# ddiazdom/grlBWT

Hardware: AMD Instinct MI355X
Metric: input MB/s building BCR BWT on 10 GB DNA reads, 1/2/4/8 MI355X (higher is better)
Workload: dtype u8; 1 GPU; 66225166 x 150 bp Illumina-style reads (10000000066 bytes) from a 330000000 bp genome, 0.5% substitutions; BASELINE configs[3]; input_resident=HBM, output=.rl_bwt image in HBM, parallelism=1 GPU

## Files before the change

### grlbwt_amd/csrc/capi_impl.hpp

```cpp
#include "../../include/grlbwt_hip.h"

#include <fcntl.h>
#include <zlib.h>
#include <sys/stat.h>
#include <unistd.h>

#include <atomic>
#include <chrono>
#include <cstdio>
#include <cstring>
#include <condition_variable>
#include <memory>
#include <mutex>
#include <string>
#include <system_error>
#include <thread>
#include <vector>


struct grlbwt_fm {
    uint32_t flags = 0;
    std::unique_ptr<grl32::Engine::FmIndex> f32;
    std::unique_ptr<grl64::Engine::FmIndex> f64;
};
// ... 1411 lines not shown
        for (uint64_t p = 0; p < n; p++) { key[p] = z[p] ? rb[j++] : ra[i++]; at[key[p] + 1]++; }
        for (int c = 0; c < 256; c++) at[c + 1] += at[c];
        for (uint64_t p = 0; p < n; p++) want[at[key[p]]++] = z[p];
    }
    grl32::DBuf<uint8_t> dra(na + 16), drb(nb + 16), dz(n + 16), dp(n + 16), dout(n + 64);
    prim::h2d(dra.p, ra.data(), na); prim::h2d(drb.p, rb.data(), nb); prim::h2d(dz.p, z.data(), n); prim::h2d(dp.p, prev.data(), n);
    prim::dev_memset(dout.p, 0xA5, n + 64);
    typename E::MergeRound W;
    W.alloc(n);
    if (W.changed(dz.p, dp.p, na) != exp_changed) return 1;
    if (W.changed(dz.p, nullptr, na) != 0) return 2;
    W.step(dra.p, drb.p, dz.p, dout.p);
    prim::sync();
    const std::vector<uint8_t> got = dout.to_host(n + 64);
    for (uint64_t p = 0; p < n; p++)
        if (got[p] != want[p]) {
            fprintf(stderr, "[grlbwt] selftest merge round: %d-byte index, %llu rows (%llu of A), %u symbols: row %llu expected flag %u, got %u\n", ib,
                    (unsigned long long)n, (unsigned long long)na, sigma, (unsigned long long)p, want[p], got[p]);
            return 3;
        }
    for (uint64_t p = n; p < n + 64; p++) if (got[p] != 0xA5) return 4;
    return 0;
}
int test_merge_round(uint64_t n, uint64_t seed) {
    const uint64_t m = self_size(n);
    const uint32_t sigmas[3] = {2, 5, 256};
    for (int k = 0; k < 3; k++) {
        if (int rc = test_merge_round_one<grl32::Engine>(m, seed + k, sigmas[k], 4)) return -(600 + rc);
        if (int rc = test_merge_round_one<grl64::Engine>(m + 1 + k, seed + 10 + k, sigmas[k], 8)) return -(610 + rc);
    }
    return 0;
}

int selftest(uint64_t n, uint64_t seed) {
    if (n < 2) n = 2;
    std::vector<uint32_t> h(n);
    uint64_t s = seed;
    for (uint64_t i = 0; i < n; i++) h[i] = (uint32_t)sm64(s);
    grl32::DBuf<uint32_t> d(n);
    prim::h2d(d.p, h.data(), n * 4);
    {
        grl32::DBuf<uint64_t> o(n + 1);
        uint64_t tot = prim::exclusive_scan<uint64_t>(n, U32In{d.p}, o.p, true, "selftest.scan");
        auto ho = o.to_host(n + 1);
        uint64_t acc = 0;
        for (uint64_t i = 0; i < n; i++) { if (ho[i] != acc) return -1; acc += h[i] & 1023u; }
        if (ho[n] != acc || tot != acc) return -2;
    }
    {
        std::vector<uint32_t> small(n);
        for (uint64_t i = 0; i < n; i++) small[i] = h[i] & 7u;
        grl32::DBuf<uint32_t> o(n);
        prim::h2d(o.p, small.data(), n * 4);
        uint32_t tot = prim::exclusive_scan<uint32_t>(n, prim::PtrIn<uint32_t>{o.p}, o.p, false, "selftest.scan32");
        auto ho = o.to_host(n);
        uint32_t acc = 0;
        for (uint64_t i = 0; i < n; i++) { if (ho[i] != acc) return -3; acc += small[i]; }
        if (tot != acc) return -4;
    }
    {
        uint64_t sum = 0; uint32_t mn = ~0u, mx = 0;
        for (uint64_t i = 0; i < n; i++) { sum += h[i] & 1023u; if (h[i] < mn) mn = h[i]; if (h[i] > mx) mx = h[i]; }
        if (prim::reduce_sum<uint64_t>(n, U32In{d.p}) != sum) return -5;
        if (prim::reduce_min<uint32_t>(n, U32Raw{d.p}) != mn) return -6;
        if (prim::reduce_max<uint32_t>(n, U32Raw{d.p}) != mx) return -7;
    }
// ... 5 lines not shown
        for (uint64_t i = 0; i < n; i++) {
            bool b = (hw[i >> 6] >> (i & 63)) & 1ull;
            if (b != ((h[i] % 3u) == 1u)) return -8;
        }
        if (n % 64) if (hw[nw - 1] >> (n % 64)) return -9;
    }
    {
        uint64_t hist[256], ref[256] = {0};
        const uint8_t *hb = (const uint8_t *)h.data();
        uint64_t nb = n * 4 - 3;
        for (uint64_t i = 0; i < nb; i++) ref[hb[i]]++;
        prim::byte_histogram((const uint8_t *)d.p, nb, hist);
        for (int i = 0; i < 256; i++) if (hist[i] != ref[i]) return -10;
    }
    { int r = test_sort<uint32_t, uint32_t>(n, seed + 1, 19); if (r) return -20 - r; }
    { int r = test_sort<uint64_t, uint32_t>(n, seed + 2, 45); if (r) return -30 - r; }
    { int r = test_sort<uint32_t, uint64_t>(n, seed + 3, 8); if (r) return -40 - r; }
    { int r = test_sort<uint64_t, uint32_t>(n, seed + 4, 3); if (r) return -50 - r; }
    { int r = test_sort<uint64_t, uint64_t>(n, seed + 5, 33); if (r) return -60 - r; }
    { int r = test_sort_keys(n, seed + 6, 21); if (r) return -90 - r; }
    { int r = test_sort<uint64_t, uint32_t>(n, seed + 7, 54); if (r) return -100 - r; }
    { int r = test_sort<uint64_t, uint32_t>(n, seed + 8, 51); if (r) return -110 - r; }
    { int r = test_sort_keys(n, seed + 9, 18); if (r) return -120 - r; }
    { int r = test_sort<uint32_t, uint64_t>(n, seed + 10, 27); if (r) return -130 - r; }
    { int r = test_sort<uint32_t, uint32_t>(n, seed + 11, 20); if (r) return -140 - r; }
    { int r = test_part(n, seed + 12, 6); if (r) return -150 - r; }
    { int r = test_part(n, seed + 13, 11); if (r) return -160 - r; }
    { int r = test_part(n, seed + 14, 18); if (r) return -170 - r; }
    { int r = test_pair_scan<uint32_t, uint32_t>(n, h, d.p); if (r) return -70 - r; }
    { int r = test_pair_scan<uint64_t, uint64_t>(n, h, d.p); if (r) return -80 - r; }
    { int r = test_stream_merge(n, seed); if (r) return r; }
#ifdef GRLBWT_PRIM_HIP
    { int r = test_seg_sort_all(seed + 40); if (r) return r; }
#endif
    { int r = test_pack(); if (r) return r; }
    { int r = test_set_bits(n, seed + 60); if (r) return r; }
    { int r = test_merge_round(n, seed + 80); if (r) return r; }
    return 0;
}

}

extern "C" {

int grlbwt_abi_version(void) { return GRLBWT_ABI_VERSION; }
const char *grlbwt_backend_name(void) { return prim::kIsDevice ? "hip-gfx950" : "serial-test-standin"; }

const char *grlbwt_strerror(int code) {
    switch (code) {
        case GRLBWT_OK: return "ok";
        case GRLBWT_EINVAL: return "invalid argument or call out of order";
        case GRLBWT_EDEVICE: return "HIP device/runtime error";
        case GRLBWT_ENOMEM: return "out of memory";
        case GRLBWT_EILLFORMED: return "Error: the file is ill formed";
        case GRLBWT_ERANGE: return "input beyond the supported range";
        case GRLBWT_ENOSPC: return "phrase table overflow";
        case GRLBWT_EINTERNAL: return "internal consistency check failed";
        case GRLBWT_ENOTDNA: return "The input seems not to be DNA";
        default: return "unknown error";
    }
}
const char *grlbwt_last_error(const grlbwt_ctx *ctx) { return ctx ? ctx->err.c_str() : ""; }

static void warn_env_switches_once() {
    static bool done = false;
    if (done) return;
// ... 87 lines not shown
    if (!ctx || !dev_in || !dev_out) return GRLBWT_EINVAL;
    return guarded(ctx, [&] {
        grl64::Engine::FastxInfo info = grl64::Engine::fastx_to_text((const uint8_t *)dev_in, n_in, (fx_flags & GRLBWT_FASTX_REVCOMP) != 0,
                                                                     (uint8_t *)dev_out, capacity);
        if (n_out) *n_out = info.n_out;
        if (n_strings) *n_strings = info.n_strings;
    });
}
int grlbwt_alphabet_size(const grlbwt_ctx *ctx, uint64_t *n_distinct) {
    if (!HAS_ENG(ctx) || !n_distinct) return GRLBWT_EINVAL;
    *n_distinct = ENG(ctx, alpha_n);
    return GRLBWT_OK;
}
int grlbwt_alphabet_download(const grlbwt_ctx *ctx, uint64_t *values_out) {
    if (!HAS_ENG(ctx) || !values_out || ENG(ctx, alpha_n) == 0) return GRLBWT_EINVAL;
    return guarded(const_cast<grlbwt_ctx *>(ctx), [&] { prim::d2h(values_out, ENG(ctx, alpha.p), ENG(ctx, alpha_n) * 8); });
}
int grlbwt_alphabet_compact_device(grlbwt_ctx *ctx, const void *dev_cells, uint64_t n_cells, int cell_bytes, void *dev_ranks_u32,
                                   void *dev_values_u64, uint64_t capacity_values, uint64_t *n_distinct) {
    if (!ctx || !dev_cells || !dev_ranks_u32 || !dev_values_u64 || n_cells == 0 || !(cell_bytes == 4 || cell_bytes == 8)) return GRLBWT_EINVAL;
    return guarded(ctx, [&] {
        const bool big = n_cells >= kIdx32Limit || (ctx->flags & GRLBWT_FLAG_FORCE_IDX64);
        uint64_t k = big ? grl64::Engine::alphabet_compact_device(dev_cells, n_cells, cell_bytes, (uint32_t *)dev_ranks_u32, (uint64_t *)dev_values_u64, capacity_values)
                         : grl32::Engine::alphabet_compact_device(dev_cells, n_cells, cell_bytes, (uint32_t *)dev_ranks_u32, (uint64_t *)dev_values_u64, capacity_values);
        if (n_distinct) *n_distinct = k;
        if (k > capacity_values) throw prim::Error(GRLBWT_EINVAL, "alphabet compaction: more distinct values than the output buffer holds");
    });
}
int grlbwt_text_load_fastx(grlbwt_ctx *ctx, const char *path, uint32_t fx_flags, uint64_t *n_strings) {
    if (!ctx || !path) return GRLBWT_EINVAL;
    return guarded(ctx, [&] { load_fastx(ctx, path, fx_flags, n_strings); });
}
int grlbwt_text_attach_device(grlbwt_ctx *ctx, const void *dev_cells, uint64_t n_cells, int cell_bytes) {
    if (!ctx || !dev_cells || ((uintptr_t)dev_cells & 15)) return GRLBWT_EINVAL;
    return guarded(ctx, [&] { load(ctx, dev_cells, n_cells, cell_bytes, false); });
}
int grlbwt_get_stats(const grlbwt_ctx *ctx, grlbwt_stats *out) {
    if (!HAS_ENG(ctx) || !out) return GRLBWT_EINVAL;
    if (ctx->e32) fill_stats(*ctx->e32, out); else fill_stats(*ctx->e64, out);
    return GRLBWT_OK;
}

int grlbwt_parse_round(grlbwt_ctx *ctx, grlbwt_round_info *info, int *done) {
    if (!HAS_ENG(ctx)) return GRLBWT_EINVAL;
    return guarded(ctx, [&] {
        bool d = ENG(ctx, parse_round());
        if (done) *done = d ? 1 : 0;
        if (info) { int r = (int)ENG(ctx, levels.size()) - 1; if (ctx->e32) fill_round(*ctx->e32, r, info); else fill_round(*ctx->e64, r, info); }
    });
}
int grlbwt_parse_phase(grlbwt_ctx *ctx, int *n_rounds) {
    if (!HAS_ENG(ctx)) return GRLBWT_EINVAL;
    return guarded(ctx, [&] { int r = ENG(ctx, parse_phase()); if (n_rounds) *n_rounds = r; });
}
int grlbwt_round_info_get(const grlbwt_ctx *ctx, int round, grlbwt_round_info *info) {
    if (!HAS_ENG(ctx) || !info || round < 0 || round >= (int)ENG(ctx, levels.size())) return GRLBWT_EINVAL;
    if (ctx->e32) fill_round(*ctx->e32, round, info); else fill_round(*ctx->e64, round, info);
    return GRLBWT_OK;
}

int grlbwt_induce_first(grlbwt_ctx *ctx) {
    if (!HAS_ENG(ctx)) return GRLBWT_EINVAL;
    return guarded(ctx, [&] { ENG(ctx, first_bwt()); });
}
int grlbwt_induce_level(grlbwt_ctx *ctx, int *level, grlbwt_level_info *info) {
    if (!HAS_ENG(ctx)) return GRLBWT_EINVAL;
    return guarded(ctx, [&] {
// ... 509 lines not shown
```

### grlbwt_amd/csrc/engine_impl.hpp

```cpp

#include "switches.hpp"

namespace GRL_NS {

using prim::u8;
using prim::u16;
using prim::u32;
using prim::u64;
typedef GRL_IDX_T idx_t;

template <class T>
struct DBuf {
    T *p = nullptr;
    u64 n = 0;
    DBuf() {}
    explicit DBuf(u64 n_) { alloc(n_); }
    DBuf(const DBuf &) = delete;
    DBuf &operator=(const DBuf &) = delete;
    DBuf(DBuf &&o) noexcept : p(o.p), n(o.n) { o.p = nullptr; o.n = 0; }
    DBuf &operator=(DBuf &&o) noexcept {
        if (this != &o) { release(); p = o.p; n = o.n; o.p = nullptr; o.n = 0; }
        return *this;
    }
    ~DBuf() { release(); }
    void alloc(u64 n_) { release(); p = (T *)prim::dev_alloc((n_ ? n_ : 1) * sizeof(T)); n = n_; }
    void release() { if (p) prim::dev_free(p); p = nullptr; n = 0; }
    void shrink(u64 n_) { if (p && n_ < n) { prim::dev_shrink(p, (n_ ? n_ : 1) * sizeof(T)); n = n_; } }
    void zero() { prim::dev_memset(p, 0, n * sizeof(T)); }
    void fill_ff() { prim::dev_memset(p, 0xFF, n * sizeof(T)); }
    std::vector<T> to_host(u64 cnt) const { std::vector<T> h(cnt); prim::d2h(h.data(), p, cnt * sizeof(T)); return h; }
    T get(u64 i) const { T v; prim::d2h(&v, p + i, sizeof(T)); return v; }
};

static inline unsigned bitlen64(u64 v) { return v == 0 ? 0 : 64 - (unsigned)__builtin_clzll(v); }

static inline bool test_fail_rank(int fail_rank, int me) {
    if constexpr (prim::kIsDevice) { (void)fail_rank; (void)me; return false; }
    else return fail_rank == me;
}

template <class T>
GRL_HD u64 upper_bound(const T *a, u64 n, T v) {
    u64 lo = 0, hi = n;
    while (lo < hi) { u64 mid = (lo + hi) >> 1; if (a[mid] <= v) lo = mid + 1; else hi = mid; }
    return lo;
}
template <class T>
GRL_HD u64 lower_bound(const T *a, u64 n, T v) {
    u64 lo = 0, hi = n;
    while (lo < hi) { u64 mid = (lo + hi) >> 1; if (a[mid] < v) lo = mid + 1; else hi = mid; }
    return lo;
}

template <class cell_t, bool FIRST>
struct CellOps {
    cell_t sep;
    GRL_HD u32 sym(cell_t c) const { return FIRST ? (u32)c : (u32)(c >> 2); }
    GRL_HD bool rep(cell_t c) const { return FIRST ? true : (bool)((c >> 1) & 1); }
    GRL_HD bool isT(cell_t c) const { return FIRST ? (c == sep) : (bool)(c & 1); }
};

GRL_HD bool bit_at(const u64 *w, u64 i) { return (w[i >> 6] >> (i & 63)) & 1ull; }
GRL_HD u64 next_set_bit(const u64 *w, u64 p, u64 n) {
    u64 r = n;
    if (p < n) {
        u64 wi = p >> 6;
        u64 x = w[wi] >> (p & 63);
        if (x) r = p + (u64)__builtin_ctzll(x);
        else {
            bool found = false;
            for (wi++; !found && (wi << 6) < n; wi++) { x = w[wi]; if (x) { r = (wi << 6) + (u64)__builtin_ctzll(x); found = true; } }
        }
        if (r > n) r = n;
    }
    return r;
}
GRL_HD u64 next_set_bit_far(const u64 *w, u64 p, u64 n) {
    u64 r = n;
    if (p < n) {
        u64 wi = p >> 6;
        u64 x = w[wi] >> (p & 63);
        if (x) r = p + (u64)__builtin_ctzll(x);
        else {
            bool found = false;
            wi++;
            bool fast = true;
            while (fast && ((wi + 8) << 6) <= n) {
                u64 any = 0;
// ... 3074 lines not shown
};

class Engine {
  public:
    ~Engine() { prim::stages_drop(); }
    int cell_bytes = 1;
    const void *text0 = nullptr;
    DBuf<u8> own0;
    DBuf<u32> rank0;
    DBuf<u64> alpha;
    u64 alpha_n = 0;
    u64 sep0() const { return alpha_n ? 0 : stats.min_sym; }
    u64 n0 = 0;
    Stats stats;
    Timers tm;
    std::vector<LevelData> levels;
    std::vector<LevelInfo> linfo;
    DBuf<u32> cur_text;
    u64 cur_n = 0;
    u32 cur_sigma = 0;
    bool parse_done = false;
    Runs bwt;
    int bwt_level = -1;
    DBuf<u8> image;
    u64 sym_present[4] = {0, 0, 0, 0};
    bool sym_present_known = false;
    u64 image_bytes = 0;
    u64 image_runs = 0;
    u64 image_part_off = 0, image_part_bytes = 0;
    bool keep_texts = false;
    std::vector<DBuf<u32>> kept_texts;
    std::vector<Runs> kept_bwts;

    template <class cell_t>
    void stats_t(const cell_t *t, u64 n, const u64 *hist256 = nullptr) {
        StageTimer st(&tm.stats, "stats");
        cell_t sep;
        prim::d2h(&sep, t + (n - 1), sizeof(cell_t));
        u64 mn, mx, F = n;
        if (sizeof(cell_t) == 1) {
            u64 h[256];
            if (hist256) std::memcpy(h, hist256, sizeof h);
            else prim::byte_histogram((const u8 *)t, n, h);
            mn = 0; while (h[mn] == 0) mn++;
            mx = 255; while (h[mx] == 0) mx--;
            F = 0; for (int i = 0; i < 256; i++) if (h[i] > F) F = h[i];
            stats.n_strings = h[(u64)sep];
            for (int i = 0; i < 4; i++) sym_present[i] = 0;
            for (int i = 0; i < 256; i++) if (h[i]) sym_present[i >> 6] |= 1ull << (i & 63);
            sym_present_known = true;
        } else {
            mn = prim::reduce_min<u64>(n, CellIn<cell_t>{t}, "stats.min");
            mx = prim::reduce_max<u64>(n, CellIn<cell_t>{t}, "stats.max");
            stats.n_strings = prim::reduce_sum<u64>(n, EqIn<cell_t>{t, sep}, "stats.nstr");
        }
        if ((u64)sep != mn) throw prim::Error(-84, "Error: the file is ill formed");
        stats.n_syms = n; stats.min_sym = mn; stats.max_sym = mx; stats.max_sym_freq = F;
        if (mx >= (1ull << 30) - 8) {
            if constexpr (sizeof(cell_t) >= 4) {
                rank0.alloc(n + 4);
                alpha_n = alphabet_compact<cell_t>(t, n, mx, rank0.p, alpha);
                if ((const void *)t == (const void *)own0.p) own0.release();
                text0 = rank0.p; cell_bytes = 4;
            }
        }
        stats.sb = (bitlen64(mx + 4) + 7) / 8;
        stats.fb = (bitlen64(F) + 7) / 8;
    }

    void load_text(const void *dev_cells, u64 n, int w, const u64 *hist256 = nullptr) {
        if (n == 0 || !(w == 1 || w == 2 || w == 4 || w == 8)) throw prim::Error(-22, "bad input size or cell width");
        if (sizeof(idx_t) == 4 && n >= 0xFFFFFF00ull) throw prim::Error(-75, "input too large for the 32-bit index build");
        if (n >= kPosMask) throw prim::Error(-75, "input too large");
        cell_bytes = w; text0 = dev_cells; n0 = n;
        prim::rt().tag = -1; prim::rt().phase = 0;
        prim::pool_reserve((size_t)(n * (u64)w) * (sizeof(idx_t) == 4 ? 22 : 30));
        levels.clear(); linfo.clear(); kept_texts.clear(); kept_bwts.clear();
        parse_done = false; bwt_level = -1; image_bytes = 0;
        rank0.release(); alpha.release(); alpha_n = 0;
        tm = Timers();
        switch (w) {
            case 1: stats_t<u8>((const u8 *)dev_cells, n, hist256); break;
            case 2: stats_t<u16>((const u16 *)dev_cells, n); break;
            case 4: stats_t<u32>((const u32 *)dev_cells, n); break;
            default: stats_t<u64>((const u64 *)dev_cells, n); break;
        }
        cur_n = n;
        cur_sigma = alpha_n ? (u32)alpha_n : (u32)(stats.max_sym + 1);
    }
    void upload_text(const void *host_cells, u64 n, int w) {
        own0.alloc(n * (u64)w + 16);
        prim::h2d(own0.p, host_cells, n * (u64)w);
        load_text(own0.p, n, w);
    }

    struct LocalParse {
        u64 n_occ = 0, D = 0, S = 0, cap = 0;
        u32 maxlen = 0;
        DBuf<u32> next_text;
        DBuf<u64> ph_pos; DBuf<idx_t> ph_freq; DBuf<u32> ph_len, ph_slot, ph_off; DBuf<u8> ph_lastT;
        u64 Ds = 0; int part_bits = 0, rec_b = 0; u32 slot0 = 0;
        DBuf<prim::U128> ph_key;
        DBuf<u32> lid, pbase;
        DBuf<u8> ph_vflag;
        DBuf<u64> pstart;
        prim::RecSort psort;
        void clear() {
            n_occ = D = S = cap = Ds = 0; maxlen = 0; part_bits = rec_b = 0; slot0 = 0;
            next_text.release(); ph_pos.release(); ph_freq.release(); ph_len.release(); ph_slot.release(); ph_off.release(); ph_lastT.release();
            ph_key.release(); ph_vflag.release(); pstart.release(); lid.release(); pbase.release(); psort.release();
        }
    };

// ... 1422 lines not shown
        while (bwt_level > 0) induce_level();
    }

    bool image_fused = false;
    void image_header(u32 sb, u32 fb) {
        u8 hdr[16] = {0};
        for (int i = 0; i < 8; i++) { hdr[i] = (u8)((u64)sb >> (8 * i)); hdr[8 + i] = (u8)((u64)fb >> (8 * i)); }
        prim::h2d(image.p, hdr, 16);
    }
    void finish() {
        if (bwt_level != 0) throw prim::Error(-22, "induction not finished");
        prim::rt().tag = -1; prim::rt().phase = 0;
        StageTimer st(&tm.finish, "finish");
        u32 sb = (u32)stats.sb, fb = (u32)stats.fb;
        if (!image_fused) {
        image_bytes = 16 + bwt.R * (u64)(sb + fb);
        image.alloc(image_bytes);
        image_header(sb, fb);
        if (sb + fb <= 8 && fb < 8) prim::pack_records(bwt.R, RunRecordFn{bwt.sym.p, run_len(), sb, alpha.p}, sb + fb, image.p + 16, "pack_rl_bwt");
        else prim::for_each(bwt.R, PackRunsFn{bwt.sym.p, run_len(), sb, fb, image.p, 16u, alpha.p}, "pack_rl_bwt");
        }
        image_fused = false;
        image_runs = bwt.R;
        image_part_off = 0; image_part_bytes = image_bytes;
        prim::sync();
    }
    u64 g_n_strings = 0, g_n_syms = 0;

    void dist_stats(const Comm &C) {
        std::vector<u64> mine(8 + 256, 0);
        mine[0] = stats.n_syms; mine[1] = stats.n_strings; mine[2] = stats.min_sym; mine[3] = stats.max_sym;
        mine[4] = sizeof(idx_t);
        if (cell_bytes == 1) {
            u64 h[256];
            prim::byte_histogram((const u8 *)text0, n0, h);
            for (int i = 0; i < 256; i++) mine[8 + i] = h[i];
        }
        std::vector<u64> all = C.allgather_u64(mine);
        const u64 w = mine.size();
        u64 n = 0, ns = 0, mn = ~0ull, mx = 0;
        std::vector<u64> hist(256, 0);
        for (int g = 0; g < C.size; g++) {
            n += all[g * w]; ns += all[g * w + 1];
            if (all[g * w + 2] < mn) mn = all[g * w + 2];
            if (all[g * w + 3] > mx) mx = all[g * w + 3];
            for (int i = 0; i < 256; i++) hist[i] += all[g * w + 8 + i];
        }
        for (int g = 0; g < C.size; g++)
            if (all[g * w + 4] != sizeof(idx_t))
                throw prim::Error(-22, "the ranks disagree on the index width: create every context with GRLBWT_FLAG_FORCE_IDX64 when the collection has >= 2^32 - 256 cells");
        for (int g = 0; g < C.size; g++)
            if (all[g * w + 2] != mn) throw prim::Error(-84, "Error: the file is ill formed");
        u64 F = n;
        if (cell_bytes == 1) { F = 0; for (int i = 0; i < 256; i++) if (hist[i] > F) F = hist[i]; }
        if (sizeof(idx_t) == 4 && n >= 0xFFFFFF00ull)
            throw prim::Error(-75, "collection too large for the 32-bit index build: create every context with GRLBWT_FLAG_FORCE_IDX64");
        if (mx >= (1ull << 30) - 8)
            throw prim::Error(-75, "symbols >= 2^30 - 8 are single-GPU for now: the collection-level mode has no global alphabet compaction yet");
        g_n_strings = ns; g_n_syms = n;
        stats.max_sym = mx; stats.max_sym_freq = F;
        stats.sb = (bitlen64(mx + 4) + 7) / 8;
        stats.fb = (bitlen64(F) + 7) / 8;
        cur_sigma = (u32)(mx + 1);
    }

    template <class cell_t, bool FIRST>
    void dist_round_t(const Comm &C, const cell_t *t, u64 n, u32 sigma, cell_t sep) {
        CellOps<cell_t, FIRST> ops{sep};
        prim::rt().tag = (int)levels.size();
// ... 1318 lines not shown
```

### grlbwt_amd/csrc/prim_hip.hpp

```cpp
#pragma once
#include <hip/hip_runtime.h>
#include <cstdint>
#include <cstdio>
#include <cstdlib>
#include <cstring>
#include <chrono>
#include <stdexcept>
#include <string>
#include <vector>
#include <map>
#include <utility>
#include <type_traits>

#define GRLBWT_PRIM_HIP 1
#include "switches.hpp"

#define GRL_HD __host__ __device__ __forceinline__
#define GRL_DEV __device__ __forceinline__

namespace prim {

typedef uint8_t u8;
typedef uint16_t u16;
typedef uint32_t u32;
// ... 671 lines not shown
                        bool fast = !ops.isT(rc);
                        while (fast && q + 4 * per + 1 < n) {
                            u64 d = 0;
#pragma unroll
                            for (int x = 0; x < 4; x++) { u64 v; __builtin_memcpy(&v, t + q + 1 + (u64)x * per, 8); d |= v ^ pat; }
                            if (d) fast = false; else q += 4 * per;
                        }
                    }
                    while (walking) {
                        const cell_t cq = t[q];
                        if (ops.isT(cq) || q + 1 >= n) walking = false;
                        else {
                            const u32 sq = ops.sym(t[q + 1]);
                            if (sq != sl) { cin = sq > sl ? 1 : 0; walking = false; }
                            else q++;
                        }
                    }
                }
                const unsigned long long Gr = __brevll(G), Pr = __brevll(P);
                const unsigned long long a = Gr | Pr, b = Gr;
                const unsigned long long s1 = a + b;
                const unsigned long long sum = s1 + cin;
                const unsigned long long ovf = ((s1 < a) || (sum < s1)) ? 1ull : 0ull;
                const unsigned long long cinto = sum ^ a ^ b;
                const unsigned long long Sr = (cinto >> 1) | (ovf << 63);
                const unsigned long long S = __brevll(Sr);
                if ((base + (u64)wv * 64) < n) words[(base >> 6) + wv] = first | (cand & S);
            }
            __builtin_amdgcn_wave_barrier();
        }
        __syncthreads();
    }
}
template <class cell_t, class OPS, class F>
inline void start_bitvector(u64 n, const cell_t *t, OPS ops, F , u64 *words, const char *name = "start_bits") {
    if (n == 0) return;
    u64 nwords = (n + 63) >> 6;
    prof_begin(name);
    (void)nwords;
    u64 ntiles = (n + (u64)kBlock * (16 / sizeof(cell_t)) - 1) / ((u64)kBlock * (16 / sizeof(cell_t)));
    u64 cap = (u64)rt().num_cus * 32;
    hipLaunchKernelGGL((k_start_bits<cell_t, OPS>), dim3((unsigned)(ntiles < cap ? ntiles : cap)), dim3(kBlock), 0, rt().stream, n, t, ops, words);
    prof_end();
    after_launch(name);
}

GRL_DEV void wave_or_words(u64 *words, bool has, u64 w, u64 m) {
    const int lane = threadIdx.x & 63;
    unsigned long long pending = __ballot(has);
    while (pending) {
        const int leader = __ffsll((long long)pending) - 1;
        const u64 wl = (u64)__shfl((unsigned long long)w, leader);
        const bool same = has && w == wl;
        unsigned long long mm = same ? (unsigned long long)m : 0ull;
#pragma unroll
        for (int off = 32; off > 0; off >>= 1) mm |= __shfl_xor(mm, off);
        if (lane == leader) atomicOr(reinterpret_cast<unsigned long long *>(&words[wl]), mm);
        pending &= ~__ballot(same);
    }
}

GRL_DEV void wave_word_store(u64 *words, u64 i, bool has) {
    const unsigned long long b = __ballot(has);
    if (b && (threadIdx.x & 63) == (unsigned)(__ffsll((long long)b) - 1)) words[i >> 6] = (u64)b;
}

static constexpr u32 kNoBucket = 0xFFFFFFFFu;
static constexpr int kAggChunk = 2048;
static constexpr u32 kDeferBucket = 0xFFFFFFFEu;
static constexpr u32 kClaimBit = 0x80000000u;
static constexpr u32 kGiantBucket = 0xFFFFFFFDu;
template <class F, class A>
__global__ void __launch_bounds__(64) k_giant(u64 n_items, const u64 *items, F f, A add) {
    const int lane = threadIdx.x & 63;
    for (u64 it = blockIdx.x; it < n_items; it += gridDim.x) {
        const u64 item = items[it];
        u64 p = 0, ee = 0;
// ... 620 lines not shown
                    if (gt == ((lo & k) == 0)) { s_k[lo] = kh; s_k[hi] = kl; s_i[lo] = ih; s_i[hi] = il; }
                }
            }
        }
        __syncthreads();
        for (u32 p = threadIdx.x; p < n; p += TB) {
            const u64 k = s_k[p];
            const bool eq_prev = p > 0 && s_k[p - 1] == k, eq_next = p + 1 < n && s_k[p + 1] == k;
            f.write(a + p, a + (u32)s_i[p], k, p > 0 && !eq_prev, eq_prev || eq_next);
        }
    }
}
template <int TB, class F>
inline void seg_sort_lds(u64 nseg, F f, u32 max_items, const char *name = "seg_sort_lds") {
    if (nseg == 0) return;
    u32 pmax = 2;
    while (pmax < max_items) pmax <<= 1;
    if (pmax > seg_sort_lds_max() || nseg > 0x7fffffffull) throw Error(-22, std::string(name) + ": segments too long or too many for the LDS sort");
    prof_begin(name);
    hipLaunchKernelGGL((k_seg_sort_lds<TB, F>), dim3((unsigned)nseg), dim3(TB), (size_t)pmax * kSegLdsItemBytes, rt().stream, f, pmax);
    prof_end();
    after_launch(name);
}

static constexpr int kHistCopies = 8;
__global__ void __launch_bounds__(kBlock) k_byte_hist(const u8 *p, u64 n, u64 *hist) {
    __shared__ u32 s_h[4][kHistCopies][257];
    for (int i = threadIdx.x; i < 4 * kHistCopies * 257; i += kBlock) (&s_h[0][0][0])[i] = 0;
    __syncthreads();
    u32 *h = s_h[threadIdx.x >> 6][threadIdx.x & (kHistCopies - 1)];
    u64 stride = (u64)gridDim.x * kBlock * 16;
    for (u64 i = ((u64)blockIdx.x * kBlock + threadIdx.x) * 16; i < n; i += stride) {
        if (i + 16 <= n) {
            uint4 v = *reinterpret_cast<const uint4 *>(p + i);
            u32 ws[4] = {v.x, v.y, v.z, v.w};
#pragma unroll
            for (int k = 0; k < 4; k++) {
                atomicAdd(&h[ws[k] & 255], 1u);
                atomicAdd(&h[(ws[k] >> 8) & 255], 1u);
                atomicAdd(&h[(ws[k] >> 16) & 255], 1u);
                atomicAdd(&h[ws[k] >> 24], 1u);
            }
        } else {
            for (u64 j = i; j < n; j++) atomicAdd(&h[p[j]], 1u);
        }
    }
    __syncthreads();
    u32 t = 0;
#pragma unroll
    for (int w = 0; w < 4; w++)
#pragma unroll
        for (int c = 0; c < kHistCopies; c++) t += s_h[w][c][threadIdx.x];
    if (t) atomicAdd(reinterpret_cast<unsigned long long *>(&hist[threadIdx.x]), (unsigned long long)t);
}
inline void byte_histogram_accumulate(const u8 *p, u64 n, u64 *d_hist) {
    if (!n) return;
    prof_begin("byte_hist");
    hipLaunchKernelGGL(k_byte_hist, dim3(grid_for(n, kBlock * 16 * 4)), dim3(kBlock), 0, rt().stream, p, n, d_hist);
    prof_end();
    after_launch("byte_hist");
}
inline void byte_histogram(const u8 *p, u64 n, u64 *hist_host) {
    u64 *d = (u64 *)dev_alloc(256 * 8);
    dev_memset(d, 0, 256 * 8);
    if (n) {
        prof_begin("byte_hist");
        hipLaunchKernelGGL(k_byte_hist, dim3(grid_for(n, kBlock * 16 * 4)), dim3(kBlock), 0, rt().stream, p, n, d);
// ... 2295 lines not shown
```

### grlbwt_amd/csrc/switches.hpp

```cpp
#pragma once
#include <cstdint>
#include <cstdlib>

#define GRLBWT_SWITCHES_PRODUCT(X)                                                                                                 \
    X(GRLBWT_PART_MIN_OCC, part_min_occ, uint64_t, (uint64_t)1 << 20, "smallest level (phrase occurrences) that takes the partitioned naming") \
    X(GRLBWT_PART_BITS, part_bits, int, 0, "partition bits of the partitioned naming, 1..20 (0: from the level's size)")          \
    X(GRLBWT_PART_ONE_PASS, part_one_pass, bool, false, "partitioned naming: records and long phrases in one pass through the table") \
    X(GRLBWT_FORCE_DIRECT_INDEX, force_direct_index, bool, false, "take the direct index on texts too small for a sample")        \
    X(GRLBWT_TABLE_TRACE, table_trace, bool, false, "trace the phrase-table and cell-layout decisions on stderr")                 \
    X(GRLBWT_A2A_SELF_VIA_COMM, a2a_self_via_comm, bool, false, "a rank's own all-to-all block goes through the callback too")    \
    X(GRLBWT_RUN_KEYS_MIN, run_keys_min, uint64_t, 512, "phrase length from which the suffix sort takes run-aware keys")         \
    X(GRLBWT_DOUBLING_AFTER, doubling_after, uint64_t, 24, "refinement rounds of a long-phrase level before doubling rounds")     \
    X(GRLBWT_SEG_CAP, seg_cap, int, 64, "largest suffix group ordered by counting (kSegCap); larger ones in LDS or by two radix sorts") \
    X(GRLBWT_SEG_LDS_CAP, seg_lds_cap, int, 4096, "largest suffix group ordered in LDS (above: two radix sorts; 0: no LDS tier)") \
    X(GRLBWT_CELL_LAYOUT, cell_layout, char, 0, "p[acked] | s[eparate]: a wider induction cell layout than the input needs")     \
    X(GRLBWT_NO_CELL32, no_cell32, bool, false, "induction cells of one word in 64 bits even where 32 would do")               \
    X(GRLBWT_ASM_TWO_PASS, asm_two_pass, bool, false, "pass C always as count + emit (no one-walk form)")                       \
    X(GRLBWT_ASM_ONE_WALK, asm_one_walk, bool, false, "pass C tries the one-walk form at every level, plain or not")           \
    X(GRLBWT_ASM_IMAGE, asm_image, int, 1, "level 0's pass C writes the .rl_bwt records itself (0: emit + pack)")             \
    X(GRLBWT_DIST_GATHERED_DICT, dist_gathered_dict, bool, false, "multi-rank: the dictionary gathered on every rank, not sharded") \
    X(GRLBWT_DIST_SHARDED_DICT_MIN, dist_sharded_dict_min, int, 4, "multi-rank: ranks from which the dictionary is sharded")    \
    X(GRLBWT_DIST_SHARDED_DICT_MIN_SYMS, dist_sharded_dict_min_syms, uint64_t, (uint64_t)1 << 27, "multi-rank: dictionary symbols from which it is sharded") \
    X(GRLBWT_INVERT, invert, char, 0, "r[uns] | p[ositions]: the form of the inversion (unset: by the memory it needs)")         \
    X(GRLBWT_XS_MAXC, xs_maxc, int, 32, "most cells per item the fused expansion sort takes (lower: the unfused branch)")        \
    X(GRLBWT_ALPHA_TABLE_BITS, alpha_table_bits, int, 20, "log2 of the slots of the alphabet compaction's table, 2..26 (lower: the sorting regime)") \
    X(GRLBWT_FM_TOP_BITS, fm_top_bits, int, 12, "log2 of the keys of an FM index's search array kept in LDS, 0..12 (0: none; lower: small indexes search HBM)") \
    X(GRLBWT_WALK_LANES, walk_lanes, uint64_t, 0, "most lanes of a checkpointed walk launch, rounded up to a wave (0: from occupancy; lower: small inputs refill their lanes)") \
    X(GRLBWT_MERGE_ROUND, merge_round, char, 0, "s[ort]: a round of the image merge as gathered keys and a stable sort, not the fused kernels") \
    X(GRLBWT_IO_THREADS, io_threads, int, 0, "reader / writer threads per file chunk, 1..64 (0: from the host's cores)")         \
    X(GRLBWT_QUIET_ENV, quiet_env, bool, false, "no note on stderr about the switches set in the environment")

#define GRLBWT_SWITCHES_INIT(X)                                                                                                     \
    X(GRLBWT_TRACE, trace, char, 0, "1: print every launch and synchronise after it")                                          \
    X(GRLBWT_SYNC_SITES, sync_sites, bool, false, "profile: count behind which launch site the host waited")                  \
    X(GRLBWT_MEM_TRACE, mem_trace, bool, false, "per-stage peak device memory on stderr")                                      \
    X(GRLBWT_NOPOOL, nopool, bool, false, "no slab allocator: hipMalloc / hipFree for every buffer")                           \
    X(GRLBWT_POOL_CLASSIC, pool_classic, bool, false, "hipMalloc slabs only, no reserved arena")                              \
    X(GRLBWT_POOL_TRACE, pool_trace, bool, false, "what backing the arena cost the process, on stderr at exit")               \
    X(GRLBWT_IO_TRACE, io_trace, bool, false, "where the file loader and the image writer spend their time, on stderr")

#define GRLBWT_SWITCHES_TEST(X)                                                                                                     \
    X(GRLBWT_NO_DIRECT_INDEX, no_direct_index, bool, false, "the hot table instead of the direct index")                       \
    X(GRLBWT_NO_HOT_TABLE, no_hot_table, bool, false, "no hot table in front of the phrase table")                            \
    X(GRLBWT_A2A_BLOCK, a2a_block, uint64_t, (uint64_t)256 << 20, "bytes of one all-to-all block before it goes in rounds")   \
    X(GRLBWT_TEST_DICT_PART_PAD, test_dict_part_pad, uint64_t, 0, "offset added to the global numbering of the dictionary parts") \
    X(GRLBWT_DIST_REC_ROUND_TRIP, dist_rec_round_trip, bool, false, "sharded sort: records travel back and forth, not carried") \
    X(GRLBWT_SORT_EXCHANGE_MIN, sort_exchange_min, int, 4, "ranks from which the sharded sort exchanges its first keys")     \
    X(GRLBWT_DIST_REC_FLY_MIN, dist_rec_fly_min, int, 8, "ranks from which the group records are made on the fly")           \
    X(GRLBWT_DIST_REPLICATED_PREBWT, dist_replicated_prebwt, bool, false, "every rank holds the whole pre-BWT")               \
    X(GRLBWT_DIST_REPLICATED_INDUCTION, dist_replicated_induction, bool, false, "the induction replicated on every rank")      \
    X(GRLBWT_DIST_REPLICATED_GRAMMAR, dist_replicated_grammar, bool, false, "the grammar passes replicated on every rank")     \
    X(GRLBWT_DIST_REPLICATED_DICT, dist_replicated_dict, bool, false, "the dictionary stage replicated on every rank")         \
    X(GRLBWT_GRAMMAR_JUMP, grammar_jump, bool, false, "the grammar walks jump to their stops whatever the phrase lengths")     \
    X(GRLBWT_MERGE_CELLS, merge_cells, char, 0, "s[ort]: the received induction cells merged by a radix sort, not by blocks") \
    X(GRLBWT_TEST_FAIL_RANK, test_fail_rank, int, -1, "this rank fails in the phrase hashing")                                \
    X(GRLBWT_TEST_FAIL_RANK_SORT, test_fail_rank_sort, int, -1, "this rank fails in the suffix refinement")                 \
    X(GRLBWT_TEST_FAIL_RANK_MERGE, test_fail_rank_merge, int, -1, "this rank fails in the phrase merge")                    \
    X(GRLBWT_TEST_FAIL_RANK_INDUCE, test_fail_rank_induce, int, -1, "this rank fails in the induction")

#define GRLBWT_SWITCHES_DEV(X)                                                                                                      \
    X(GRLBWT_NO_PART, no_part, bool, false, "no partitioned naming (single GPU)")                                              \
    X(GRLBWT_DIST_NO_PART, dist_no_part, bool, false, "no partitioned naming (multi-rank)")                                   \
    X(GRLBWT_NO_NAME_STREAM, no_name_stream, bool, false, "the direct index without the name_stream kernel")                  \
    X(GRLBWT_SORT_KMAX, sort_kmax, int, 16, "most symbols in the first suffix sort's key")                                     \
    X(GRLBWT_FOR_EACH_GRID, for_each_grid, char, 0, "f[ixed]: 8 workgroups per CU; anything else: twice the resident number") \
    X(GRLBWT_SPAN_BLOCKS_PER_CU, span_blocks_per_cu, uint64_t, 0, "workgroups per CU of the span kernels (0: from occupancy)") \
// ... 75 lines not shown
```

Measured before the change: 13800 MB/s.

## Add SWAR byte-wise phrase-start bitvector kernel for level-0 u8 texts

Adds a dedicated kernel for the level-0 phrase-start (LMS-like) bitvector on byte texts. Each lane loads 16 bytes at a time and builds compare masks with SWAR byte tricks and udot4 packing. Masks are exchanged across lanes with DPP and shuffles, and the S/L type propagation is resolved with a reversed carry-add instead of a per-cell scan, walking ahead only for runs that cross a word. It also caches the byte histogram computed in stats so the distributed path does not recompute it, and relaxes the alignment check for byte inputs. The risk is correctness on long runs and boundary cases, which a new self-test covers.

```diff
diff --git a/grlbwt_amd/csrc/capi_impl.hpp b/grlbwt_amd/csrc/capi_impl.hpp
--- a/grlbwt_amd/csrc/capi_impl.hpp
+++ b/grlbwt_amd/csrc/capi_impl.hpp
@@ -1467,6 +1467,135 @@
     return 0;
 }
 
+#ifdef GRLBWT_PRIM_HIP
+struct SbText { std::vector<uint8_t> c; uint8_t sep = 0; const char *what = ""; };
+std::vector<uint64_t> sb_reference(const std::vector<uint8_t> &t, uint8_t sep) {
+    const uint64_t n = t.size();
+    std::vector<uint64_t> w((n + 63) / 64, 0);
+    bool s_next = false;
+    for (uint64_t p = n; p-- > 0;) {
+        const bool T = t[p] == sep;
+        const bool S = !T && p + 1 < n && (t[p + 1] > t[p] || (t[p + 1] == t[p] && s_next));
+        if (p == 0 || t[p - 1] == sep || (t[p - 1] > t[p] && S)) w[p >> 6] |= 1ull << (p & 63);
+        s_next = S;
+    }
+    return w;
+}
+int test_start_bits_one(const SbText &x, int behind, bool with_pred, double *ms_new = nullptr, double *ms_generic = nullptr) {
+    const uint64_t n = x.c.size(), nw = (n + 63) / 64, stride = nw + 2;
+    grl32::DBuf<uint8_t> dt(n + 64);
+    grl32::DBuf<uint64_t> dw(3 * stride);
+    uint8_t *t = dt.p + ((16 - (uintptr_t)dt.p % 16) % 16) + behind;
+    prim::h2d(t, x.c.data(), n);
+    prim::dev_memset(dw.p, 0xA5, 3 * stride * 8);
+    const grl32::CellOps<uint8_t, true> ops{x.sep};
+    auto timed = [&](double *ms, auto launch) {
+        if (ms) prim::sync();
+        const auto t0 = std::chrono::steady_clock::now();
+        launch();
+        if (ms) { prim::sync(); *ms = std::chrono::duration<double>(std::chrono::steady_clock::now() - t0).count() * 1e3; }
+    };
+    timed(ms_new, [&] { prim::start_bitvector_u8(n, t, x.sep, dw.p, "selftest.start_bits_u8"); });
+    timed(ms_generic, [&] { prim::start_bitvector_generic(n, (const uint8_t *)t, ops, dw.p + stride, "selftest.start_bits"); });
+    if (with_pred) prim::bitvector_from_pred(n, grl32::StartPred<uint8_t, true>{t, ops}, dw.p + 2 * stride, "selftest.start_pred");
+    const std::vector<uint64_t> got = dw.to_host(3 * stride), want = sb_reference(x.c, x.sep);
+    for (int k = 0; k < 3; k++) {
+        const uint64_t *o = got.data() + k * stride;
+        if ((k < 2 || with_pred) && (o[nw] != 0xA5A5A5A5A5A5A5A5ull || o[nw + 1] != 0xA5A5A5A5A5A5A5A5ull)) return 4;
+    }
+    for (uint64_t w = 0; w < nw; w++) {
+        const uint64_t g = got[w], refs[3] = {want[w], with_pred ? got[2 * stride + w] : want[w], got[stride + w]};
+        for (int k = 0; k < 3; k++)
+            if (g != refs[k]) {
+                const uint64_t p = w * 64 + (uint64_t)__builtin_ctzll(g ^ refs[k]);
+                char cells[128]; int len = 0;
+                for (uint64_t q = p >= 6 ? p - 6 : 0; q < n && q < p + 7; q++) len += snprintf(cells + len, sizeof cells - len, q == p ? " [%02x]" : " %02x", x.c[q]);
+                fprintf(stderr, "[grlbwt] selftest start bits (u8): %s, %llu cells, separator %02x, %d bytes behind a 16-byte boundary: word %llu is %016llx, %s has %016llx; "
+                        "first at position %llu, cells%s\n", x.what, (unsigned long long)n, x.sep, behind, (unsigned long long)w, (unsigned long long)g,
+                        k == 0 ? "the host" : k == 1 ? "StartPred" : "k_start_bits", (unsigned long long)refs[k], (unsigned long long)p, cells);
+                return 1 + k;
+            }
+    }
+    return 0;
+}
+int test_start_bits(uint64_t seed) {
+    uint64_t s = seed;
+    std::vector<SbText> texts;
+    const uint64_t lens[9] = {1, 2, 63, 64, 65, 4095, 4096, 4097, 65537};
+    const char *anames[5] = {"{0; 1..4}", "ACGTN", "all 256 values", "{7f; 80..ff}", "{7f, 80, ff}"};
+    for (uint64_t n : lens)
+        for (int a = 0; a < 5; a++) {
+            SbText x; x.what = anames[a];
+            x.sep = a == 1 ? (uint8_t)'\n' : (a >= 3 ? 0x7F : 0);
+            auto cell = [&]() -> uint8_t {
+                const uint64_t r = sm64(s);
+                if (r % 23 == 0) return x.sep;
+                switch (a) {
+                    case 0: return (uint8_t)(1 + (r >> 8) % 4);
+                    case 1: return (uint8_t)"ACGTN"[(r >> 8) % 5];
+                    case 2: return (uint8_t)(r >> 8);
+                    case 3: return (uint8_t)(0x80 + (r >> 8) % 128);
+                    default: return (uint8_t)((r >> 8) % 3 == 0 ? 0x7F : ((r >> 8) % 3 == 1 ? 0x80 : 0xFF));
+                }
+            };
+            while (x.c.size() + 1 < n) {
+                const uint8_t c = cell();
+                uint64_t rep = sm64(s) % 4 == 0 ? 1 + sm64(s) % 70 : 1;
+                for (; rep && x.c.size() + 1 < n; rep--) x.c.push_back(c);
+            }
+            x.c.push_back(x.sep);
+            texts.push_back(std::move(x));
+        }
+    {
+        SbText x; x.what = "{7f, 80, ff} in every order"; x.sep = 0x7F;
+        const uint8_t v[3] = {0x7F, 0x80, 0xFF};
+        for (int i = 0; i < 27; i++) { x.c.push_back(v[i % 3]); x.c.push_back(v[i / 3 % 3]); x.c.push_back(v[i / 9]); x.c.push_back(0x80); }
+        x.c.push_back(x.sep);
+        texts.push_back(std::move(x));
+    }
+    for (int shift : {0, 3, 5}) {
+        SbText x; x.what = "runs of 1..200"; x.sep = 0;
+        for (int i = 0; i < shift; i++) x.c.push_back(i % 2 ? 1 : 3);
+        for (int L = 1; L <= 200; L++)
+            for (int before : {3, 1})
+                for (int after : {3, 1, 0}) { x.c.push_back((uint8_t)before); x.c.insert(x.c.end(), L, 2); x.c.push_back((uint8_t)after); }
+        x.c.push_back(3); x.c.insert(x.c.end(), 77, 2); x.c.push_back(0);
+        texts.push_back(std::move(x));
+    }
+    {
+        SbText x; x.what = "runs on the boundaries"; x.sep = 0;
+        int i = 0;
+        for (uint64_t B : {8, 16, 64, 1024, 4096})
+            for (uint64_t L : {1, 2, 3, 15, 16, 17, 63, 64, 65, 130, 200})
+                for (uint64_t off : {(uint64_t)1, L / 2, L - 1, L})
+                    for (int before : {3, 1}) {
+                        while ((x.c.size() + 1 + off) % B != 0) x.c.push_back(x.c.size() % 2 ? 1 : 3);
+                        x.c.push_back((uint8_t)before); x.c.insert(x.c.end(), L, 2); x.c.push_back((uint8_t)(i % 3 == 0 ? 3 : (i % 3 == 1 ? 1 : 0)));
+                        i++;
+                    }
+        x.c.push_back(0);
+        texts.push_back(std::move(x));
+    }
+    {   SbText x; x.what = "adjacent separators"; x.sep = 0; x.c = {0, 0, 2, 1, 0, 0, 0, 1, 2, 2, 0, 0}; x.c.insert(x.c.end(), 130, 0); texts.push_back(std::move(x)); }
+    {   SbText x; x.what = "one string"; x.sep = 0; for (int i = 0; i < 5000; i++) x.c.push_back((uint8_t)(1 + sm64(s) % 4)); x.c.push_back(0); texts.push_back(std::move(x)); }
+    for (const SbText &x : texts)
+        for (int behind : {0, 1, 7, 15})
+            if (int rc = test_start_bits_one(x, behind, true)) return -(700 + rc);
+    for (int after : {3, 1}) {
+        SbText x; x.what = "a run of 3,000,000"; x.sep = 0;
+        x.c = {1, 0, 1, 3}; x.c.insert(x.c.end(), 3000000, 2); x.c.push_back((uint8_t)after); x.c.push_back(0);
+        double ms_new = 0, ms_generic = 0;
+        if (int rc = test_start_bits_one(x, 1, false, &ms_new, &ms_generic)) return -(720 + rc);
+        if (prim::init_sw().trace) fprintf(stderr, "[grlbwt] selftest start bits (u8): a run of 3,000,000 cells: %.3f ms (k_start_bits: %.3f ms)\n", ms_new, ms_generic);
+        if (ms_new > 4 * ms_generic + 5) {
+            fprintf(stderr, "[grlbwt] selftest start bits (u8): a run of 3,000,000 cells took %.3f ms, k_start_bits %.3f ms\n", ms_new, ms_generic);
+            return -719;
+        }
+    }
+    return 0;
+}
+#endif
+
 int selftest(uint64_t n, uint64_t seed) {
     if (n < 2) n = 2;
     std::vector<uint32_t> h(n);
@@ -1538,6 +1667,7 @@
     { int r = test_stream_merge(n, seed); if (r) return r; }
 #ifdef GRLBWT_PRIM_HIP
     { int r = test_seg_sort_all(seed + 40); if (r) return r; }
+    { int r = test_start_bits(seed + 90); if (r) return r; }
 #endif
     { int r = test_pack(); if (r) return r; }
     { int r = test_set_bits(n, seed + 60); if (r) return r; }
@@ -1691,7 +1821,7 @@
     return guarded(ctx, [&] { load_fastx(ctx, path, fx_flags, n_strings); });
 }
 int grlbwt_text_attach_device(grlbwt_ctx *ctx, const void *dev_cells, uint64_t n_cells, int cell_bytes) {
-    if (!ctx || !dev_cells || ((uintptr_t)dev_cells & 15)) return GRLBWT_EINVAL;
+    if (!ctx || !dev_cells || (cell_bytes != 1 && ((uintptr_t)dev_cells & 15))) return GRLBWT_EINVAL;
     return guarded(ctx, [&] { load(ctx, dev_cells, n_cells, cell_bytes, false); });
 }
 int grlbwt_get_stats(const grlbwt_ctx *ctx, grlbwt_stats *out) {
diff --git a/grlbwt_amd/csrc/engine_impl.hpp b/grlbwt_amd/csrc/engine_impl.hpp
--- a/grlbwt_amd/csrc/engine_impl.hpp
+++ b/grlbwt_amd/csrc/engine_impl.hpp
@@ -54,6 +54,7 @@
 
 template <class cell_t, bool FIRST>
 struct CellOps {
+    static constexpr bool kFirst = FIRST;
     cell_t sep;
     GRL_HD u32 sym(cell_t c) const { return FIRST ? (u32)c : (u32)(c >> 2); }
     GRL_HD bool rep(cell_t c) const { return FIRST ? true : (bool)((c >> 1) & 1); }
@@ -3194,6 +3195,9 @@
     std::vector<DBuf<u32>> kept_texts;
     std::vector<Runs> kept_bwts;
 
+    u64 hist0[256];
+    bool hist0_known = false;
+
     template <class cell_t>
     void stats_t(const cell_t *t, u64 n, const u64 *hist256 = nullptr) {
         StageTimer st(&tm.stats, "stats");
@@ -3201,9 +3205,10 @@
         prim::d2h(&sep, t + (n - 1), sizeof(cell_t));
         u64 mn, mx, F = n;
         if (sizeof(cell_t) == 1) {
-            u64 h[256];
-            if (hist256) std::memcpy(h, hist256, sizeof h);
+            u64 *const h = hist0;
+            if (hist256) std::memcpy(h, hist256, sizeof hist0);
             else prim::byte_histogram((const u8 *)t, n, h);
+            hist0_known = true;
             mn = 0; while (h[mn] == 0) mn++;
             mx = 255; while (h[mx] == 0) mx--;
             F = 0; for (int i = 0; i < 256; i++) if (h[i] > F) F = h[i];
@@ -3241,6 +3246,7 @@
         parse_done = false; bwt_level = -1; image_bytes = 0;
         rank0.release(); alpha.release(); alpha_n = 0;
         tm = Timers();
+        hist0_known = false;
         switch (w) {
             case 1: stats_t<u8>((const u8 *)dev_cells, n, hist256); break;
             case 2: stats_t<u16>((const u16 *)dev_cells, n); break;
@@ -4729,9 +4735,8 @@
         mine[0] = stats.n_syms; mine[1] = stats.n_strings; mine[2] = stats.min_sym; mine[3] = stats.max_sym;
         mine[4] = sizeof(idx_t);
         if (cell_bytes == 1) {
-            u64 h[256];
-            prim::byte_histogram((const u8 *)text0, n0, h);
-            for (int i = 0; i < 256; i++) mine[8 + i] = h[i];
+            if (!hist0_known) { prim::byte_histogram((const u8 *)text0, n0, hist0); hist0_known = true; }
+            for (int i = 0; i < 256; i++) mine[8 + i] = hist0[i];
         }
         std::vector<u64> all = C.allgather_u64(mine);
         const u64 w = mine.size();
diff --git a/grlbwt_amd/csrc/prim_hip.hpp b/grlbwt_amd/csrc/prim_hip.hpp
--- a/grlbwt_amd/csrc/prim_hip.hpp
+++ b/grlbwt_amd/csrc/prim_hip.hpp
@@ -727,17 +727,168 @@
         __syncthreads();
     }
 }
-template <class cell_t, class OPS, class F>
-inline void start_bitvector(u64 n, const cell_t *t, OPS ops, F , u64 *words, const char *name = "start_bits") {
-    if (n == 0) return;
-    u64 nwords = (n + 63) >> 6;
+GRL_DEV u32 sb8_zero_bytes(u32 z) {
+    return ~(((z & 0x7f7f7f7fu) + 0x7f7f7f7fu) | z) & 0x80808080u;
+}
+GRL_DEV u32 sb8_ge_bytes(u32 a, u32 b) {
+    const u32 d = (a | 0x80808080u) - (b & 0x7f7f7f7fu);
+    return ((a & ~b) | (~(a ^ b) & d)) & 0x80808080u;
+}
+GRL_DEV u32 sb8_dot(u32 bytes, u32 weights, u32 acc) {
+#if __has_builtin(__builtin_amdgcn_udot4)
+    return __builtin_amdgcn_udot4(bytes, weights, acc, false);
+#else
+    for (int b = 0; b < 4; b++) acc += ((bytes >> (8 * b)) & 255u) * ((weights >> (8 * b)) & 255u);
+    return acc;
+#endif
+}
+GRL_DEV void sb8_load16(const u8 *t, u64 q, u64 n, u32 (&w)[4]) {
+    if (q + 16 <= n) __builtin_memcpy(w, t + q, 16);
+    else {
+        u64 lo = 0, hi = 0;
+#pragma unroll 1
+        for (u64 j = 0; j < 16 && q + j < n; j++) {
+            const u64 c = t[q + j];
+            if (j < 8) lo |= c << (8 * j); else hi |= c << (8 * (j - 8));
+        }
+        w[0] = (u32)lo; w[1] = (u32)(lo >> 32); w[2] = (u32)hi; w[3] = (u32)(hi >> 32);
+    }
+}
+__global__ void __launch_bounds__(kBlock) k_start_bits_u8(u64 n, const u8 *t, u8 sep, u64 *words) {
+    constexpr int LOADS = 4;
+    constexpr u64 WTILE = 64 * 16 * LOADS;
+    const int lane = threadIdx.x & 63;
+    const u64 ntiles = (n + WTILE - 1) / WTILE;
+    const u64 nwaves = (u64)gridDim.x * (kBlock / 64);
+    const u32 sep4 = (u32)sep * 0x01010101u;
+    for (u64 tile = (u64)blockIdx.x * (kBlock / 64) + (threadIdx.x >> 6); tile < ntiles; tile += nwaves) {
+        const u64 base = tile * WTILE;
+        u32 v[LOADS][4];
+        u32 before = 0, behind = 0;
+        if (base > 0 && base + WTILE < n) {
+#pragma unroll
+            for (int k = 0; k < LOADS; k++) __builtin_memcpy(v[k], t + base + (u64)k * 1024 + (u64)lane * 16, 16);
+            before = (u32)t[base - 1]; behind = (u32)t[base + WTILE];
+        } else {
+#pragma unroll
+            for (int k = 0; k < LOADS; k++) sb8_load16(t, base + (u64)k * 1024 + (u64)lane * 16, n, v[k]);
+            if (base > 0) before = (u32)t[base - 1];
+            if (base + WTILE < n) behind = (u32)t[base + WTILE];
+        }
+        const u32 edge0 = before << 24, edge1 = (u32)__builtin_amdgcn_readlane((int)v[0][3], 63), edge2 = (u32)__builtin_amdgcn_readlane((int)v[1][3], 63),
+                  edge3 = (u32)__builtin_amdgcn_readlane((int)v[2][3], 63);
+        const u32 last = (u32)__builtin_amdgcn_readlane((int)v[3][3], 63) >> 24;
+        u32 nxt = (last > behind ? 1u : 0u) | (last == behind ? 0x10000u : 0u);
+#pragma unroll 1
+        for (int k = LOADS - 1; k >= 0; k--) {
+            u32 cw[4];
+#pragma unroll
+            for (int x = 0; x < 4; x++) cw[x] = k == 0 ? v[0][x] : (k == 1 ? v[1][x] : (k == 2 ? v[2][x] : v[3][x]));
+            u32 pw = (u32)__shfl_up((int)cw[3], 1);
+            if (lane == 0) pw = k == 0 ? edge0 : (k == 1 ? edge1 : (k == 2 ? edge2 : edge3));
+            u32 ma = 0, me = 0, mt = 0, mah = 0, meh = 0, mth = 0;
+#pragma unroll
+            for (int x = 0; x < 4; x++) {
+                const u32 c = cw[x];
+                const u32 pv = (c << 8) | ((x ? cw[x > 0 ? x - 1 : 0] : pw) >> 24);
+                const u32 e = sb8_zero_bytes(pv ^ c);
+                const u32 a = sb8_ge_bytes(pv, c) & ~e;
+                const u32 tt = sb8_zero_bytes(c ^ sep4);
+                const u32 wts = (x & 1) ? 0x80402010u : 0x08040201u;
+                if (x < 2) { ma = sb8_dot(a, wts, ma); me = sb8_dot(e, wts, me); mt = sb8_dot(tt, wts, mt); }
+                else { mah = sb8_dot(a, wts, mah); meh = sb8_dot(e, wts, meh); mth = sb8_dot(tt, wts, mth); }
+            }
+            ma |= mah << 8; me |= meh << 8; mt |= mth << 8;
+            const u32 r0 = ((ma >> 7) & 0xffffu) | ((me >> 7) << 16);
+            const u32 r1 = ((mt >> 7) & 0xffffu) | ((pw >> 24) == (u32)sep ? 0x10000u : 0u);
+            u32 nx = (u32)__shfl_down((int)r0, 4);
+            if (lane >= 60) nx = nxt;
+            nxt = (u32)__builtin_amdgcn_readfirstlane((int)r0);
+            const u32 r0b = (u32)__builtin_amdgcn_mov_dpp((int)r0, 0xF9, 0xf, 0xf, true), r1b = (u32)__builtin_amdgcn_mov_dpp((int)r1, 0xF9, 0xf, 0xf, true);
+            const u32 r0c = (u32)__builtin_amdgcn_mov_dpp((int)r0, 0xFE, 0xf, 0xf, true), r1c = (u32)__builtin_amdgcn_mov_dpp((int)r1, 0xFE, 0xf, 0xf, true);
+            const u32 r0d = (u32)__builtin_amdgcn_mov_dpp((int)r0, 0xFF, 0xf, 0xf, true), r1d = (u32)__builtin_amdgcn_mov_dpp((int)r1, 0xFF, 0xf, 0xf, true);
+            const u64 wp = base + (u64)k * 1024 + (u64)(lane >> 2) * 64;
+            if ((lane & 3) == 0 && wp < n) {
+                const unsigned long long A = (u64)((r0 & 0xffffu) | (r0b << 16)) | ((u64)((r0c & 0xffffu) | (r0d << 16)) << 32);
+                const unsigned long long E = (u64)((r0 >> 16) | (r0b & 0xffff0000u)) | ((u64)((r0c >> 16) | (r0d & 0xffff0000u)) << 32);
+                const unsigned long long T = (u64)((r1 & 0xffffu) | (r1b << 16)) | ((u64)((r1c & 0xffffu) | (r1d << 16)) << 32);
+                const u64 left = n - wp;
+                const unsigned long long inm = left >= 64 ? ~0ull : (1ull << left) - 1ull;
+                const unsigned long long nxm = left >= 65 ? ~0ull : (1ull << (left - 1)) - 1ull;
+                const unsigned long long An = (A >> 1) | ((u64)(nx & 1u) << 63), En = (E >> 1) | ((u64)((nx >> 16) & 1u) << 63);
+                const unsigned long long open = nxm & ~T;
+                const unsigned long long G = open & ~(An | En), P = open & En;
+                const unsigned long long p0 = wp == 0 ? 1ull : 0ull;
+                const unsigned long long first = inm & ((T << 1) | (u64)((r1 >> 16) & 1u) | p0);
+                const unsigned long long cand = inm & A & ~p0;
+                unsigned long long cin = 0;
+                const int trailing = (~P == 0ull) ? 64 : __builtin_clzll(~P);
+                const int rstart = 64 - trailing;
+                if ((P >> 63) && ((cand >> rstart) & 1ull)) {
+                    const u32 sl = (u32)t[wp + 63];
+                    u64 q = wp + 64;
+                    bool walking = true;
+                    {
+                        const u8 rc = t[q];
+                        const u64 pat = (u64)rc * 0x0101010101010101ull;
+                        bool fast = rc != sep;
+                        while (fast && q + 33 < n) {
+                            u64 d = 0;
+#pragma unroll
+                            for (int x = 0; x < 4; x++) { u64 w; __builtin_memcpy(&w, t + q + 1 + (u64)x * 8, 8); d |= w ^ pat; }
+                            if (d) fast = false; else q += 32;
+                        }
+                    }
+                    while (walking) {
+                        const u8 cq = t[q];
+                        if (cq == sep || q + 1 >= n) walking = false;
+                        else {
+                            const u32 sq = (u32)t[q + 1];
+                            if (sq != sl) { cin = sq > sl ? 1 : 0; walking = false; }
+                            else q++;
+                        }
+                    }
+                }
+                const unsigned long long Gr = __brevll(G), Pr = __brevll(P);
+                const unsigned long long a = Gr | Pr, b = Gr;
+                const unsigned long long s1 = a + b;
+                const unsigned long long sum = s1 + cin;
+                const unsigned long long ovf = ((s1 < a) || (sum < s1)) ? 1ull : 0ull;
+                const unsigned long long cinto = sum ^ a ^ b;
+                const unsigned long long Sr = (cinto >> 1) | (ovf << 63);
+                const unsigned long long S = __brevll(Sr);
+                words[wp >> 6] = first | (cand & S);
+            }
+        }
+    }
+}
+template <class OPS>
+constexpr auto start_bits_first_level(int) -> decltype(OPS::kFirst) { return OPS::kFirst; }
+template <class OPS>
+constexpr bool start_bits_first_level(long) { return false; }
+inline void start_bitvector_u8(u64 n, const u8 *t, u8 sep, u64 *words, const char *name) {
+    const u64 wtiles = (n + 4095) / 4096, blocks = (wtiles + kBlock / 64 - 1) / (kBlock / 64), cap = (u64)rt().num_cus * 32;
     prof_begin(name);
-    (void)nwords;
+    hipLaunchKernelGGL(k_start_bits_u8, dim3((unsigned)(blocks < cap ? blocks : cap)), dim3(kBlock), 0, rt().stream, n, t, sep, words);
+    prof_end();
+    after_launch(name);
+}
+template <class cell_t, class OPS>
+inline void start_bitvector_generic(u64 n, const cell_t *t, OPS ops, u64 *words, const char *name) {
+    prof_begin(name);
     u64 ntiles = (n + (u64)kBlock * (16 / sizeof(cell_t)) - 1) / ((u64)kBlock * (16 / sizeof(cell_t)));
     u64 cap = (u64)rt().num_cus * 32;
     hipLaunchKernelGGL((k_start_bits<cell_t, OPS>), dim3((unsigned)(ntiles < cap ? ntiles : cap)), dim3(kBlock), 0, rt().stream, n, t, ops, words);
     prof_end();
     after_launch(name);
+}
+template <class cell_t, class OPS, class F>
+inline void start_bitvector(u64 n, const cell_t *t, OPS ops, F , u64 *words, const char *name = "start_bits") {
+    if (n == 0) return;
+    if constexpr (sizeof(cell_t) == 1 && start_bits_first_level<OPS>(0)) {
+        if (sw().text_scan >= 1) { start_bitvector_u8(n, (const u8 *)t, (u8)ops.sep, words, name); return; }
+    }
+    start_bitvector_generic(n, t, ops, words, name);
 }
 
 GRL_DEV void wave_or_words(u64 *words, bool has, u64 w, u64 m) {
@@ -1424,7 +1575,8 @@
     u64 stride = (u64)gridDim.x * kBlock * 16;
     for (u64 i = ((u64)blockIdx.x * kBlock + threadIdx.x) * 16; i < n; i += stride) {
         if (i + 16 <= n) {
-            uint4 v = *reinterpret_cast<const uint4 *>(p + i);
+            uint4 v;
+            __builtin_memcpy(&v, p + i, 16);
             u32 ws[4] = {v.x, v.y, v.z, v.w};
 #pragma unroll
             for (int k = 0; k < 4; k++) {
diff --git a/grlbwt_amd/csrc/switches.hpp b/grlbwt_amd/csrc/switches.hpp
--- a/grlbwt_amd/csrc/switches.hpp
+++ b/grlbwt_amd/csrc/switches.hpp
@@ -27,11 +27,12 @@
     X(GRLBWT_FM_TOP_BITS, fm_top_bits, int, 12, "log2 of the keys of an FM index's search array kept in LDS, 0..12 (0: none; lower: small indexes search HBM)") \
     X(GRLBWT_WALK_LANES, walk_lanes, uint64_t, 0, "most lanes of a checkpointed walk launch, rounded up to a wave (0: from occupancy; lower: small inputs refill their lanes)") \
     X(GRLBWT_MERGE_ROUND, merge_round, char, 0, "s[ort]: a round of the image merge as gathered keys and a stable sort, not the fused kernels") \
+    X(GRLBWT_TEXT_SCAN, text_scan, int, 1, "level 0 of a byte text: 1: the byte-wise phrase-start kernel; 0: the generic one")   \
     X(GRLBWT_IO_THREADS, io_threads, int, 0, "reader / writer threads per file chunk, 1..64 (0: from the host's cores)")         \
     X(GRLBWT_QUIET_ENV, quiet_env, bool, false, "no note on stderr about the switches set in the environment")
 
 #define GRLBWT_SWITCHES_INIT(X)                                                                                                     \
-    X(GRLBWT_TRACE, trace, char, 0, "1: print every launch and synchronise after it")                                          \
+    X(GRLBWT_TRACE, trace, char, 0, "1: print every launch and synchronise after it; another value: the timings the self-test takes") \
     X(GRLBWT_SYNC_SITES, sync_sites, bool, false, "profile: count behind which launch site the host waited")                  \
     X(GRLBWT_MEM_TRACE, mem_trace, bool, false, "per-stage peak device memory on stderr")                                      \
     X(GRLBWT_NOPOOL, nopool, bool, false, "no slab allocator: hipMalloc / hipFree for every buffer")                           \
```

Result: no change. 13800 MB/s (-0.0%).
